# TinyMPC/TinyMPC

Measured on AMD Instinct MI355X. Metric: QP solves/sec (+ ADMM iters/sec), 64k-batch quadrotor hover, higher is better.
Workload: dtype f64; 1 GPU; quadrotor_hovering (nx=12, nu=4, N=10), 65536 identical instances per GPU, closed-loop MPC steps from a cold start (BASELINE configs[1]); batch_per_gpu=65536, total_batch=65536, parallelism=batch-sharded x1, mpc_steps_per_launch=8, stats_exchange=none (one rank), launcher=plain process

## Files before the change

tinympc_amd/csrc/admm_kernel.hip.h:

```cpp
#pragma once
#include <hip/hip_runtime.h>
#include <stdint.h>

namespace tinympc_amd {

enum : int {
    TAB_MB = 0,
    TAB_MF1 = 256,
    TAB_MF2 = 512,
    TAB_PT = 768,
    TAB_VEC = 1024,
    TAB_BOUNDS = 1024 + 16 * 16,
};
enum : int {
    VEC_CB = 0,
    VEC_CF = 1,
    VEC_QR = 2,
    VEC_SMASK = 3,
    VEC_NIM = 4,
    VEC_SOCFLAG = 5,
    VEC_CONE_BASE = 6,
    VEC_CONE_MU = 7,
    VEC_LINFLAG = 9,
    VEC_TLINFLAG = 10,
    VEC_COUNT = 16,
};
enum : int { LIN_KMAX = 4, LIN_KMAX_BIG = 32 };
enum : int {
    ATAB_AT = 0,
    ATAB_DK = 256,
    ATAB_DP = 512,
    ATAB_DC1 = 768,
    ATAB_DC2 = 1024,
    ATAB_DOUBLES = 1280,
};
// ... 293 lines not shown
    return r;
}
__device__ __forceinline__ double pinned_sub64(double a, double b) {
    double r = a - b;
    asm volatile("" : "+v"(r));
    return r;
}
__device__ __forceinline__ double vclamp64(double lo, double hi, double t) {
    double r;
    asm("v_max_f64 %0, %1, %2\n\tv_min_f64 %0, %3, %0" : "=&v"(r) : "v"(lo), "v"(t), "v"(hi));
    return r;
}

__device__ __forceinline__ double vmax_abs64(double a, double b) {
    double r;
    asm("v_max_f64 %0, %1, |%2|" : "=v"(r) : "v"(a), "v"(b));
    return r;
}
template <bool OPAQUE>
__device__ __forceinline__ double resid_max(double a, double b) {
    if constexpr (OPAQUE) return vmax_abs64(a, b);
    else return fmax(a, fabs(b));
}

#ifndef TINYMPC_PRIM_STORE
#define TINYMPC_PRIM_STORE 1
#endif
#ifndef TINYMPC_REF_LOAD
#define TINYMPC_REF_LOAD 1
#endif
#ifndef TINYMPC_FULL_LINE_STORES
#define TINYMPC_FULL_LINE_STORES 2
#endif
__device__ __forceinline__ double load_ref(const double* p) {
#if TINYMPC_REF_LOAD == 1
    return __builtin_nontemporal_load(p);
#else
    return *p;
#endif
}
__device__ __forceinline__ void store_primal(double* p, double v) {
#if TINYMPC_PRIM_STORE == 1
    __builtin_nontemporal_store(v, p);
#elif TINYMPC_PRIM_STORE == 2
    asm volatile("global_store_dwordx2 %0, %1, off sc1" : : "v"(p), "v"(v) : "memory");
#elif TINYMPC_PRIM_STORE == 3
    asm volatile("global_store_dwordx2 %0, %1, off sc0 sc1" : : "v"(p), "v"(v) : "memory");
#elif TINYMPC_PRIM_STORE == 4
    asm volatile("global_store_dwordx2 %0, %1, off sc0 sc1 nt" : : "v"(p), "v"(v) : "memory");
#else
    *p = v;
#endif
}

__device__ __forceinline__ double grp_max16(double v) {
#pragma unroll
    for (int off = 8; off >= 1; off >>= 1) v = fmax(v, __shfl_xor(v, off, 16));
    return v;
}
template <int W>
__device__ __forceinline__ double grp_maxw(double v) {
#pragma unroll
    for (int off = W / 2; off >= 1; off >>= 1) v = fmax(v, __shfl_xor(v, off, W));
    return v;
}

// ... 95 lines not shown
            double cv = 0.0;
#pragma unroll
            for (int r = 0; r < NF; ++r) { const double pr = tk[k * LW_ + R0 + r] * z[r]; cv = cv + pr; }
            const double bk = tk[KMAX_ * LW_ + k * LW_ + R0];
            if (cv > bk) {
                const double dist = (cv - bk) / tk[2 * KMAX_ * LW_ + k * LW_ + R0];
#pragma unroll
                for (int r = 0; r < NF; ++r) { const double pr = dist * tk[k * LW_ + R0 + r]; z[r] = z[r] - pr; }
            }
        }
#pragma unroll
        for (int r = 0; r < NF; ++r) { pv[at + r] = z[r]; pg[at + r] = t0[r] - z[r]; }
    }
}

template <int NX, int NU, int N, bool SOC, bool DBG, int MODE, int LIN = 0, bool HET = false, int KMAX = LIN_KMAX, bool ADAPT = false, bool UB = false, bool HALF = false,
          bool PF = false>
__global__ __launch_bounds__(64)
__attribute__((amdgpu_waves_per_eu(LIN != 0 ? solve_kernel_lin_waves(NX, NU, N, SOC, LIN, KMAX, UB) : solve_kernel_waves_per_simd(NX + NU, N, SOC, false, ADAPT),
                                   LIN != 0 ? solve_kernel_lin_waves(NX, NU, N, SOC, LIN, KMAX, UB) : solve_kernel_waves_per_simd(NX + NU, N, SOC, false, ADAPT))))
void admm_solve_kernel(const SolveArgs P) {
    constexpr bool LS = (LIN & 1) != 0, LT = (LIN & 2) != 0;
    constexpr int NZ = NX + NU;
    static_assert(NZ <= 16, "one instance per 16-lane DPP row");
    constexpr bool FUSED = MODE == 2 && LIN == 0 && fused_shape(NX, NU);
    static_assert(!HALF || (NZ <= 8 && FUSED && !SOC && !DBG && !HET && !ADAPT), "half rows: nx+nu <= 8, the plain box kernel on its fused step blocks");
    static_assert(!PF || (MODE == 2 && !SOC && !DBG && LIN == 0 && !HET && !ADAPT), "prefetch form: the plain box kernel");
    constexpr int RL = HALF ? 8 : 16;
    constexpr int IPW = 64 / RL;
    constexpr int RECD = N * NZ;
    constexpr int PF_PIECES = (IPW * RECD * 8 + 1023) / 1024;
    constexpr int PF_ARR = PF_PIECES * 128;
    constexpr unsigned long long RMASK = HALF ? 0xFFull : 0xFFFFull;
    const int lane = threadIdx.x & 63;
    const int j = lane & (RL - 1);
    const int grp = lane / RL;
    const bool is_state = j < NX;
    const bool is_input = (j >= NX) && (j < NZ);

    __shared__ double sPt[NX * 16];
    __shared__ double sLo[UB ? 1 : N * 16];
    __shared__ double sHi[UB ? 1 : N * 16];
    __shared__ double sLin[LS ? 3 * KMAX * 16 : 1];
    __shared__ double sTLin[LT ? 3 * N * KMAX * 16 : 1];
#ifndef TINYMPC_SOC_PD
#define TINYMPC_SOC_PD 2
#endif
    constexpr int SPD = TINYMPC_SOC_PD, SPR = SPD + 1;
    constexpr int CS = SOC ? ((NZ + 1) | 1) : 1;
    constexpr int SLOT_D = 3 * CS;
    constexpr int PL_GC = CS, PL_VC = 2 * CS;
    __shared__ double sC[SOC ? (4 * N + 1) * SLOT_D : 1];
    __shared__ double sP[ADAPT ? 4 * NX * NX : 1];
    constexpr int AKC = NX > NU ? NX : NU;
    constexpr bool HA = HET && ADAPT;
    __shared__ double sTab[(ADAPT && !HET) ? 3 * 16 * AKC : 1];
    __shared__ double sDl[ADAPT ? 4 * ADAPT_LOG : 1];
    if constexpr (ADAPT && !HET)
        for (int e = lane; e < 3 * 16 * AKC; e += 64) {
            const int t = e / (16 * AKC), r = e % (16 * AKC);
            sTab[e] = P.atab[t * 256 + (r % AKC) * 16 + r / AKC];
        }
    if constexpr (LS) for (int e = lane; e < 3 * KMAX * 16; e += 64) sLin[e] = P.tab[TAB_BOUNDS + 2 * N * 16 + e];
    if constexpr (LT) for (int e = lane; e < 3 * N * KMAX * 16; e += 64) sTLin[e] = P.tab[TAB_BOUNDS + 2 * N * 16 + 3 * KMAX * 16 + e];
    for (int e = lane; e < NX * 16; e += 64) sPt[e] = P.tab[TAB_PT + e];
    for (int e = lane; e < N * 16; e += 64) {
        if constexpr (!UB) {
            sLo[e] = P.tab[TAB_BOUNDS + e];
            sHi[e] = P.tab[TAB_BOUNDS + N * 16 + e];
        }
    }
    double mb[NZ], mf1[NX], mf2[NU];
#pragma unroll
    for (int k = 0; k < NZ; ++k) mb[k] = P.tab[TAB_MB + k * 16 + j];
#pragma unroll
// ... 32 lines not shown
            int t = p * 16 + j;
            item_at[p] = 4 * N * SLOT_D; item_mu[p] = 1.0f;
            if (heads && p * 16 < soc_items_of(heads, NX, N)) soc_passes = p + 1;
            for (unsigned m = heads; m; m &= m - 1) {
                const int hb = __builtin_ctz(m);
                const int cnt = hb < NX ? N : N - 1;
                if (t >= 0 && t < cnt) {
                    item_at[p] = (grp * N + t + (hb < NX ? 0 : 1)) * SLOT_D + hb;
                    item_mu[p] = (float)P.tab[TAB_VEC + VEC_CONE_MU * 16 + hb];
                    t = -1;
                } else if (t >= 0) t -= cnt;
            }
            item_rmu[p] = 1.0f / item_mu[p];
            const unsigned mb_ = __float_as_uint(item_mu[p]);
            const bool p2 = (mb_ & 0x807FFFFFu) == 0u && (mb_ >> 23) >= 127u - 60u && (mb_ >> 23) <= 127u + 60u;
            if (__builtin_amdgcn_ballot_w64(!p2) != 0ull) mu_pow2 = false;
        }
    }
    bool lin_lane = false, tlin_lane = false;
    if constexpr (LS) lin_lane = P.tab[TAB_VEC + VEC_LINFLAG * 16 + j] != 0.0;
    if constexpr (LT) tlin_lane = P.tab[TAB_VEC + VEC_TLINFLAG * 16 + j] != 0.0;
    constexpr bool LPL = solve_kernel_lin_planes(NX, NU, N, SOC, LIN, KMAX, UB);
    constexpr bool LSP = LS && LPL, LTP = LT && LPL, LSR = LS && !LPL, LTR = LT && !LPL;
    constexpr int CSL = LPL ? ((NZ + 1) | 1) : 1;
    __shared__ double sLV[LSP ? 4 * N * CSL : 1], sLG[LSP ? 4 * N * CSL : 1];
    __shared__ double sTV[LTP ? 4 * N * CSL : 1], sTG[LTP ? 4 * N * CSL : 1];
    double ones[(LSR || LTR) ? 16 : 1];
#pragma unroll
    for (int k = 0; k < ((LSR || LTR) ? 16 : 1); ++k) ones[k] = 1.0;
    bool lin_x_on = false, lin_u_on = false, tlin_x_on = false, tlin_u_on = false;
    if constexpr (LS) { lin_x_on = P.tab[TAB_VEC + VEC_LINFLAG * 16] != 0.0; lin_u_on = P.tab[TAB_VEC + VEC_LINFLAG * 16 + NX] != 0.0; }
    if constexpr (LT) { tlin_x_on = P.tab[TAB_VEC + VEC_TLINFLAG * 16] != 0.0; tlin_u_on = P.tab[TAB_VEC + VEC_TLINFLAG * 16 + NX] != 0.0; }
    double rho = P.rho;
    __builtin_amdgcn_fence(__ATOMIC_RELEASE, "wavefront");
    __builtin_amdgcn_wave_barrier();

    const double lo_u = P.tab[TAB_BOUNDS + (N > 1 ? 16 : 0) + j], hi_u = P.tab[TAB_BOUNDS + N * 16 + (N > 1 ? 16 : 0) + j];
    const double lo_u0 = P.tab[TAB_BOUNDS + j], hi_u0 = P.tab[TAB_BOUNDS + N * 16 + j];
    const int ninst = PF ? P.batch : (P.index ? *P.count : (P.perm ? P.perm_count : P.batch));
    const int ntiles = (ninst + IPW - 1) / IPW;
    const bool resumed = !PF && P.index != nullptr;
    const bool has_traj = !PF && P.traj != nullptr;
    extern __shared__ __attribute__((aligned(16))) double sPF[];
    typedef const __attribute__((address_space(1))) void* pf_gptr;
    typedef __attribute__((address_space(3))) void* pf_lptr;
    constexpr int PF_S0 = 128, PF_S1 = PF_S0 + PF_ARR, PF_S2 = PF_S1 + PF_ARR, PF_S3 = PF_S2 + PF_ARR;
    auto pf_issue = [&](const int t) {
        const int tl = P.reverse ? ntiles - 1 - t : t;
        __builtin_amdgcn_global_load_lds((pf_gptr)(P.x0 + ((size_t)tl * (IPW * NX) + (size_t)lane * 2)), (pf_lptr)sPF, 16, 0, 0);
        const size_t t0 = (size_t)tl * (IPW * RECD) + (size_t)lane * 2;
        auto arr = [&](const double* p, const int at) {
#pragma unroll
            for (int q = 0; q < PF_PIECES; ++q) __builtin_amdgcn_global_load_lds((pf_gptr)(p + t0 + q * 128), (pf_lptr)(sPF + at + q * 128), 16, 0, 0);
        };
        if (!P.cold) { arr(P.slack, PF_S0); arr(P.dual, PF_S1); arr(P.slack_prev, PF_S2); }
        if (P.pf_mask & 8) arr(P.ref, P.cold ? PF_S0 : PF_S3);
    };
    unsigned pf_ticket = 0u;
    const int pf_shard = PF ? (int)(blockIdx.x % (unsigned)(P.pf_shards > 0 ? P.pf_shards : 1)) : 0;
    typedef __attribute__((address_space(1))) unsigned* pf_ctr_t;
    unsigned long long pf_ctr_bits = PF ? (unsigned long long)(P.pf_counter + 16 * pf_shard) : 0ull;
    if constexpr (PF) asm volatile("" : "+v"(pf_ctr_bits));
    const pf_ctr_t pf_ctr = (pf_ctr_t)pf_ctr_bits;
    auto pf_draw = [&]() { return lane == 0 ? __hip_atomic_fetch_add(pf_ctr, 1u, __ATOMIC_RELAXED, __HIP_MEMORY_SCOPE_AGENT) : 0u; };
    const unsigned pf_base = PF ? P.pf_base[pf_shard] : 0u;
    int pf_next = 0, pf_i = 0;
// ... 87 lines not shown
            const double* het = nullptr;
            if constexpr (HET) {
                het = P.het_tabs + (size_t)b * TAB_BOUNDS;
#pragma unroll
                for (int k = 0; k < NZ; ++k) mb[k] = het[TAB_MB + k * 16 + j];
#pragma unroll
                for (int k = 0; k < NX; ++k) mf1[k] = het[TAB_MF1 + k * 16 + j];
#pragma unroll
                for (int k = 0; k < NU; ++k) mf2[k] = het[TAB_MF2 + (NX + k) * 16 + j];
                cb = het[TAB_VEC + VEC_CB * 16 + j];
                cf = het[TAB_VEC + VEC_CF * 16 + j];
                qr = het[TAB_VEC + VEC_QR * 16 + j];
                rho = het[TAB_VEC + 8 * 16 + j];
            }
            if constexpr (ADAPT) {
                rho = P.arho[b];
                const double* aK = P.aK + (size_t)b * (NU * NX);
                if (is_state) {
#pragma unroll
                    for (int k = 0; k < NU; ++k) mb[NX + k] = -aK[k + NU * j];
#pragma unroll
                    for (int k = 0; k < NX; ++k) sP[grp * NX * NX + k + NX * j] = P.aP[(size_t)b * (NX * NX) + k + NX * j];
                } else if (is_input) {
#pragma unroll
                    for (int k = 0; k < NX; ++k) mf1[k] = -aK[(j - NX) + NU * k];
                }
                __builtin_amdgcn_fence(__ATOMIC_RELEASE, "wavefront");
                __builtin_amdgcn_wave_barrier();
            }
            const double* atab_i = nullptr;
            if constexpr (HET && ADAPT) atab_i = P.atab + (size_t)b * ATAB_DOUBLES;
            (void)atab_i;
            const size_t lbase = (size_t)b * (N * NZ) + j - (is_input ? NZ : 0);
            double X[N], G[N], VN[N], VP[N], QX[N], Dn[N - 1];
            const int cw = grp * N * SLOT_D + (j < NZ ? j : NZ);
            const double x0v_in = is_state ? (PF ? pf_x0 : P.x0[(size_t)b * NX + j]) : 0.0;
            const int cl = grp * N * CSL + (j < NZ ? j : NZ);
            double VL[LSR ? N : 1], GL[LSR ? N : 1], VT[LTR ? N : 1], GT[LTR ? N : 1];
            double Qd[DBG ? N : 1], Pd[DBG ? N : 1], Dd[DBG ? N : 1];
            double ref_last = 0.0, qx_last_plain = 0.0;
#pragma unroll
            for (int s = 0; s < N; ++s) {
                const bool valid = is_state || (is_input && s >= 1);
                const size_t off = lbase + s * NZ;
                const bool warm = valid && !P.cold;
                if constexpr (PF) {
                    VN[s] = warm ? pfVN[s] : 0.0;
                    G[s] = warm ? pfG[s] : 0.0;
                    VP[s] = warm ? pfVP[s] : 0.0;
                    QX[s] = pfQXs[s];
                    X[s] = 0.0;
                    if (s == N - 1) ref_last = pf_rl;
                    continue;
                }
                const double r = valid ? (P.ref_shared ? P.ref[off - (size_t)b * (N * NZ)] : load_ref(P.ref + off)) : 0.0;
                VN[s] = warm ? P.slack[off] : 0.0;
                G[s] = warm ? P.dual[off] : 0.0;
                VP[s] = warm ? P.slack_prev[off] : 0.0;
                QX[s] = -(r * qr);
                X[s] = 0.0;
                if (s == N - 1) ref_last = r;
                if constexpr (SOC) {
                    double vc0 = (warm && soc_lane) ? (resumed ? P.cslack : P.prim)[off] : 0.0;
                    const double gc0 = (warm && soc_lane) ? P.cdual[off] : 0.0;
                    if (s == 0 && is_state && soc_lane && !resumed) vc0 = x0v_in;
                    sC[cw + s * SLOT_D] = vc0 - gc0;
                    sC[cw + s * SLOT_D + PL_GC] = gc0;
                    sC[cw + s * SLOT_D + PL_VC] = vc0;
                }
                if constexpr (LS) {
                    const double vl0 = (warm && lin_lane) ? (resumed ? P.lslack : P.prim)[off] : 0.0;
                    const double gl0 = (warm && lin_lane) ? P.ldual[off] : 0.0;
                    if constexpr (LSP) { sLV[cl + s * CSL] = vl0; sLG[cl + s * CSL] = gl0; } else { VL[s] = vl0; GL[s] = gl0; }
                }
                if constexpr (LT) {
                    const double vt0 = (warm && tlin_lane) ? (resumed ? P.tlslack : P.prim)[off] : 0.0;
                    const double gt0 = (warm && tlin_lane) ? P.tldual[off] : 0.0;
                    if constexpr (LTP) { sTV[cl + s * CSL] = vt0; sTG[cl + s * CSL] = gt0; } else { VT[s] = vt0; GT[s] = gt0; }
                }
                if constexpr (DBG) { Qd[s] = 0.0; Pd[s] = 0.0; Dd[s] = 0.0; }
            }
            double x0v = x0v_in;
            auto terminal_term = [&]() {
                double pt[NX];
#pragma unroll
                for (int k = 0; k < NX; ++k)
                    pt[k] = ADAPT ? sP[grp * NX * NX + k + NX * (is_state ? j : 0)] : (HET ? het[TAB_PT + k * 16 + j] : sPt[k * 16 + j]);
                double xp = 0.0;
                if constexpr (HALF) ring1_half<0, NX>(xp, ref_last, pt);
                else xp = ring_sum<MODE, 0, NX>(0.0, ref_last, pt);
                qx_last_plain = QX[N - 1];
// ... 3 lines not shown
            auto flush_c = [&](int n) {
                __builtin_amdgcn_fence(__ATOMIC_RELEASE, "wavefront");
                __builtin_amdgcn_wave_barrier();
                if (P.aC2 && is_state) {
                    double* c2 = P.aC2 + (size_t)b * (NX * NX) + NX * j;
                    double v[NX], d[NX];
#pragma unroll
                    for (int k = 0; k < NX; ++k) { v[k] = c2[k]; d[k] = P.atab[(HA ? (size_t)b * ATAB_DOUBLES : (size_t)0) + ATAB_DC2 + k * 16 + j]; }
                    for (int i = 0; i < n; ++i) {
                        const double dl = sDl[grp * ADAPT_LOG + i];
#pragma unroll
                        for (int k = 0; k < NX; ++k) v[k] = taylor_step(v[k], dl, d[k]);
                    }
#pragma unroll
                    for (int k = 0; k < NX; ++k) c2[k] = v[k];
                }
                if (P.aC1 && j < NU) {
                    double* c1 = P.aC1 + (size_t)b * (NU * NU) + NU * j;
                    double v[NU], d[NU];
#pragma unroll
                    for (int k = 0; k < NU; ++k) { v[k] = c1[k]; d[k] = P.atab[(HA ? (size_t)b * ATAB_DOUBLES : (size_t)0) + ATAB_DC1 + k * 16 + j]; }
                    for (int i = 0; i < n; ++i) {
                        const double dl = sDl[grp * ADAPT_LOG + i];
#pragma unroll
                        for (int k = 0; k < NU; ++k) v[k] = taylor_step(v[k], dl, d[k]);
                    }
#pragma unroll
                    for (int k = 0; k < NU; ++k) c1[k] = v[k];
                }
            };
            if (!has_traj && !(PF && P.ref_shared)) terminal_term();
            const int traj_k0 = has_traj ? (P.traj_step0 + (P.traj_offsets ? P.traj_offsets[b] : 0)) : 0;

            int iter = 0, solved = 0, checked = 0;
            unsigned acc_iter = 0, acc_solved = 0;
            bool vp_touched = false;
            double rp = 0.0, rd = 0.0;
            const int nsteps = PF ? 1 : (P.steps > 1 ? P.steps : 1);
            const int iter_first = resumed ? P.iter_base : 0;
            for (int step = 0; step < nsteps; ++step) {
                X[0] = x0v;
                if (has_traj) {
                    if (is_state) {
#pragma unroll
                        for (int s = 0; s < N; ++s) {
                            int kk = traj_k0 + step + s;
                            kk = kk < P.traj_points ? kk : P.traj_points - 1;
                            const double r = P.traj[(size_t)kk * NX + j];
                            QX[s] = -(r * qr);
                            if (s == N - 1) ref_last = r;
                        }
                    }
                    terminal_term();
                }
                if (P.reset_duals) {
#pragma unroll
                    for (int s = 0; s < N; ++s) G[s] = 0.0;
                }
                if constexpr (SOC) {
                    if (step > 0) {
#pragma unroll
                        for (int s = 0; s < N; ++s) {
                            const double vc0 = soc_lane ? X[s] : 0.0;
                            sC[cw + s * SLOT_D] = vc0 - sC[cw + s * SLOT_D + PL_GC];
                            sC[cw + s * SLOT_D + PL_VC] = vc0;
                        }
                    }
                }
                if constexpr (LS) {
                    if (step > 0) {
#pragma unroll
                        for (int s = 0; s < N; ++s) { if constexpr (LSP) sLV[cl + s * CSL] = lin_lane ? X[s] : 0.0; else VL[s] = lin_lane ? X[s] : 0.0; }
                    } else if (is_state && lin_lane && !resumed) { if constexpr (LSP) sLV[cl] = x0v; else VL[0] = x0v; }
                }
                if constexpr (LT) {
                    if (step > 0) {
#pragma unroll
                        for (int s = 0; s < N; ++s) { if constexpr (LTP) sTV[cl + s * CSL] = tlin_lane ? X[s] : 0.0; else VT[s] = tlin_lane ? X[s] : 0.0; }
                    } else if (is_state && tlin_lane && !resumed) { if constexpr (LTP) sTV[cl] = x0v; else VT[0] = x0v; }
                }
                if constexpr (LPL) __builtin_amdgcn_fence(__ATOMIC_RELEASE, "wavefront");
                const int iter0 = iter_first;
                iter = iter0; solved = 0;
                if (resumed && P.check_termination > 0) checked = 1;
                int countdown = P.check_termination;
                double wr[SOC ? SPR : 1];
                bool gcz[SOC_PASSES];
#pragma unroll
                for (int p = 0; p < SOC_PASSES; ++p) gcz[p] = false;
                if constexpr (SOC) {
#pragma unroll
                    for (int d = 1; d <= SPR && d <= N; ++d) wr[(N - d) % SPR] = sC[cw + (N - d) * SLOT_D];
                }
                for (int it = iter0; it < P.max_iter; ++it) {
                    double lvr[LSP ? SPR : 1], lgr[LSP ? SPR : 1], tvr[LTP ? SPR : 1], tgr[LTP ? SPR : 1];
                    if constexpr (LPL) {
#pragma unroll
                        for (int d = 1; d <= SPR && d <= N; ++d) {
                            if constexpr (LSP) { lvr[(N - d) % SPR] = sLV[cl + (N - d) * CSL]; lgr[(N - d) % SPR] = sLG[cl + (N - d) * CSL]; }
                            if constexpr (LTP) { tvr[(N - d) % SPR] = sTV[cl + (N - d) * CSL]; tgr[(N - d) % SPR] = sTG[cl + (N - d) * CSL]; }
                        }
                    }
                    auto lin_w = [&](const int s_) { if constexpr (LSP) return lvr[s_ % SPR] - lgr[s_ % SPR]; else return VL[LSR ? s_ : 0] - GL[LSR ? s_ : 0]; };
                    auto tlin_w = [&](const int s_) { if constexpr (LTP) return tvr[s_ % SPR] - tgr[s_ % SPR]; else return VT[LTR ? s_ : 0] - GT[LTR ? s_ : 0]; };
                    double qhi;
                    {
                        double t = fma(-rho, VN[N - 1] - G[N - 1], QX[N - 1]);
                        if constexpr (SOC) t = fma(-rho, wr[(N - 1) % SPR], t);
                        if constexpr (LS) t = fma(-rho, lin_w(N - 1), t);
                        if constexpr (LT) t = fma(-rho, tlin_w(N - 1), t);
                        qhi = t;
                        if constexpr (DBG) {
                            double ql = fma(-rho, VN[N - 1] - G[N - 1], qx_last_plain);
                            if constexpr (SOC) ql = fma(-rho, wr[(N - 1) % SPR], ql);
                            if constexpr (LS) ql = fma(-rho, lin_w(N - 1), ql);
                            if constexpr (LT) ql = fma(-rho, tlin_w(N - 1), ql);
                            Qd[N - 1] = is_state ? ql : t;
                            Pd[N - 1] = t;
// ... 13 lines not shown
                            pcur = res;
                            qhi = qlo;
                        }
                        Dn[0] = fma(pcur, nim, cf);
                    }
#pragma unroll
                    for (int i = N - 2; i >= 0 && !HALF; --i) {
                        if constexpr (SOC) {
                            if (i >= SPD) wr[(i - SPD) % SPR] = sC[cw + (i - SPD) * SLOT_D];
                        }
                        if constexpr (LSP) { if (i >= SPD) { lvr[(i - SPD) % SPR] = sLV[cl + (i - SPD) * CSL]; lgr[(i - SPD) % SPR] = sLG[cl + (i - SPD) * CSL]; } }
                        if constexpr (LTP) { if (i >= SPD) { tvr[(i - SPD) % SPR] = sTV[cl + (i - SPD) * CSL]; tgr[(i - SPD) % SPR] = sTG[cl + (i - SPD) * CSL]; } }
                        if constexpr (SOC || LPL) __builtin_amdgcn_sched_barrier(0);
                        if constexpr (FUSED) {
                            double qlo, res;
                            if constexpr (SOC) fused_backward_step_soc<NX, NU>(qlo, res, VN[i], G[i], QX[i], wr[i % SPR], rho, smask, cb, pcur, qhi, mb, mb + NX);
                            else fused_backward_step<NX, NU>(qlo, res, VN[i], G[i], QX[i], rho, smask, cb, pcur, qhi, mb, mb + NX);
                            pcur = res;
                            Dn[i] = fma(res, nim, cf);
                            if constexpr (DBG) { Qd[i] = qlo; Pd[i] = res; Dd[i + 1] = res; }
                            qhi = qlo;
                            continue;
                        }
                        double qlo = fma(-rho, VN[i] - G[i], QX[i]);
                        if constexpr (SOC) qlo = fma(-rho, wr[i % SPR], qlo);
                        if constexpr (LS) qlo = fma(-rho, lin_w(i), qlo);
                        if constexpr (LT) qlo = fma(-rho, tlin_w(i), qlo);
                        const double res = ring_sum2<MODE, NX, NU>(fma(qlo, smask, cb), pcur, mb, qhi, mb + NX);
                        pcur = res;
                        Dn[i] = fma(res, nim, cf);
                        if constexpr (DBG) { Qd[i] = qlo; Pd[i] = res; Dd[i + 1] = res; }
                        qhi = qlo;
                    }
                    constexpr bool LAZY_RES = N <= 12;
                    constexpr bool TIGHT = FUSED && !HALF && LAZY_RES && !SOC && NX % 4 == 0;
                    double pmax = 0.0, dmax = 0.0;
                    auto slot_update = [&](const int s, const double lo, const double hi, const double gcv, const double glv, const double gtv) {
                        const double xi = X[s];
                        const double t = xi + G[s];
                        const double vn = TIGHT ? vclamp64(lo, hi, t) : vmin64(hi, vmax64(lo, t));
                        if constexpr (!LAZY_RES) {
                            pmax = resid_max<true>(pmax, xi - vn);
                            dmax = resid_max<true>(dmax, VP[s] - vn);
                        }
                        G[s] = t - vn;
                        VN[s] = vn;
                        if constexpr (SOC) {
                            sC[cw + s * SLOT_D] = fma(xi, socmask, gcv);
                        }
                        if constexpr (LSP) sLV[cl + s * CSL] = (lin_lane && (is_state || s >= 1)) ? (xi + glv) : 0.0;
                        if constexpr (LTP) sTV[cl + s * CSL] = (tlin_lane && (is_state || s >= 1)) ? (xi + gtv) : 0.0;
                        if constexpr (LSR || LTR) {
                            auto halfspaces = [&](double z, const double* tabk, const int nk) {
                                for (int k = 0; k < nk; ++k) {
                                    const double a = tabk[k * 16 + j];
                                    const double bk = tabk[KMAX * 16 + k * 16 + j];
                                    const double nn = tabk[2 * KMAX * 16 + k * 16 + j];
                                    const double prod = a * z;
                                    double cs = 0.0, ci = 0.0;
                                    ring1<0, NX>(cs, prod, ones);
                                    ring1<NX, NU>(ci, prod, ones);
                                    const double cv = is_state ? cs : ci;
                                    if (cv > bk) z = z - ((cv - bk) / nn) * a;
                                }
                                return z;
                            };
                            if constexpr (LSR) {
                                const bool on = lin_lane && (is_state || s >= 1);
// ... 62 lines not shown
                                tt_d = tt; vn_d = vn;
                            } else G[i] = tt - vn;
                            VN[i] = vn;
                            if constexpr (SOC) sC[cw + i * SLOT_D] = fma(xi, socmask, gr[i % SPR]);
                            lo_c = lo_n; hi_c = hi_n;
                            continue;
                        }
                        const double t = ring_sum<MODE, 0, NX>(Dn[i], X[i], mf1);
                        X[i + 1] = ring_short<MODE, NX, NU>(t, t, mf2);
                        slot_update(i, lo_c, hi_c, gr[SOC ? i % SPR : 0], glr[LSP ? i % SPR : 0], gtr[LTP ? i % SPR : 0]);
                        lo_c = lo_n; hi_c = hi_n;
                    }
                    if constexpr (TIGHT && N >= 2) G[N - 2] = tt_d - vn_d;
                    (void)tt_d; (void)vn_d;
                    slot_update(N - 1, lo_c, hi_c, gr[SOC ? (N - 1) % SPR : 0], glr[LSP ? (N - 1) % SPR : 0], gtr[LTP ? (N - 1) % SPR : 0]);
                    if constexpr (LPL) {
                        __builtin_amdgcn_fence(__ATOMIC_RELEASE, "wavefront");
                        __builtin_amdgcn_wave_barrier();
                        if constexpr (LSP) {
                            if (lin_x_on) project_halfspace_columns<NX, KMAX, 16, 16>(j, grp, N, CSL, 0, 0, sLV, sLG, sLin, 0, P.n_lin);
                            if (lin_u_on) project_halfspace_columns<NU, KMAX, 16, 16>(j, grp, N, CSL, NX, 1, sLV, sLG, sLin, 0, P.n_lin);
                        }
                        if constexpr (LTP) {
                            if (tlin_x_on) project_halfspace_columns<NX, KMAX, 16, 16>(j, grp, N, CSL, 0, 0, sTV, sTG, sTLin, 3 * KMAX * 16, P.n_tlin);
                            if (tlin_u_on) project_halfspace_columns<NU, KMAX, 16, 16>(j, grp, N, CSL, NX, 1, sTV, sTG, sTLin, 3 * KMAX * 16, P.n_tlin);
                        }
                        __builtin_amdgcn_fence(__ATOMIC_RELEASE, "wavefront");
                        __builtin_amdgcn_wave_barrier();
                    }
                    bool conv = false;
                    auto termination = [&]() {
                        if (countdown > 0 && --countdown == 0) {
                            countdown = P.check_termination;
                            checked = 1;
                            constexpr int PS0 = N >= 2 ? 1 : 0, PS1 = N - 1;
                            auto lost = [&](const int s) {
                                return (int)(fabs(X[s] - VN[s]) >= P.tol_pri) | (int)(fabs(VP[s] - VN[s]) * rho >= P.tol_dua);
                            };
                            const bool maybe = ((int)!(rho > 0.0) | (int)!(lost(PS0) | lost(PS1))) != 0;
                            unsigned long long fold = __ballot(maybe);
                            fold &= fold >> 1; fold &= fold >> 2; fold &= fold >> 4;
                            if constexpr (!HALF) fold &= fold >> 8;
                            const bool any_row = (fold & (HALF ? 0x0101010101010101ull : 0x0001000100010001ull)) != 0ull;
                            const bool last_test = (P.max_iter - 1 - it) < P.check_termination;
                            if (last_test || any_row) {
                                if constexpr (LAZY_RES) {
#pragma unroll
                                    for (int s = 0; s < N; ++s) {
                                        pmax = resid_max<false>(pmax, X[s] - VN[s]);
                                        dmax = resid_max<false>(dmax, VP[s] - VN[s]);
                                    }
                                }
                                rp = pmax;
                                rd = dmax * rho;
                                const bool ok = (rp < P.tol_pri) && (rd < P.tol_dua);
                                const unsigned long long bal = __ballot(ok);
                                conv = ((bal >> (grp * RL)) & RMASK) == RMASK;
                            }
                        }
                    };
                    if constexpr (SOC) {
                        __builtin_amdgcn_fence(__ATOMIC_RELEASE, "wavefront");
                        __builtin_amdgcn_wave_barrier();
                        double n0 = sC[item_at[0]], n1 = sC[item_at[0] + 1], n2 = sC[item_at[0] + 2];
#pragma unroll
                        for (int d = 1; d <= SPR && d <= N; ++d) wr[(N - d) % SPR] = sC[cw + (N - d) * SLOT_D];
                        termination();
                        bool any_exact = false;
#pragma unroll
                        for (int p = 0; p < SOC_PASSES; ++p) {
                            if (p > 0 && p >= soc_passes) break;
                            const int at = item_at[p];
                            if (p > 0) { n0 = sC[at]; n1 = sC[at + 1]; n2 = sC[at + 2]; }
                            const double s0 = n0, s1 = n1, s2 = n2;
                            if (soc_all_inside(s0, s1, s2, item_mu[p])) {
                                sC[at + PL_VC] = s0; sC[at + PL_VC + 1] = s1; sC[at + PL_VC + 2] = s2;
                                if (!gcz[p]) {
                                    sC[at + PL_GC] = 0.0; sC[at + PL_GC + 1] = 0.0; sC[at + PL_GC + 2] = 0.0;
                                    gcz[p] = true;
                                }
                            } else {
                                double r0, r1, r2;
                                soc_project3(s0, s1, s2, item_mu[p], item_rmu[p], mu_pow2, r0, r1, r2);
                                const double g0 = s0 - r0, g1 = s1 - r1, g2 = s2 - r2;
                                sC[at + PL_VC] = r0; sC[at + PL_VC + 1] = r1; sC[at + PL_VC + 2] = r2;
                                sC[at + PL_GC] = g0; sC[at + PL_GC + 1] = g1; sC[at + PL_GC + 2] = g2;
                                sC[at] = r0 - g0; sC[at + 1] = r1 - g1; sC[at + 2] = r2 - g2;
                                gcz[p] = false;
                                any_exact = true;
                            }
                        }
                        if (it == iter0 && !proj_lane) {
#pragma unroll
                            for (int s = 0; s < N; ++s) sC[cw + s * SLOT_D + PL_GC] = 0.0;
                        }
                        __builtin_amdgcn_fence(__ATOMIC_RELEASE, "wavefront");
                        __builtin_amdgcn_wave_barrier();
                        if (any_exact) {
#pragma unroll
                            for (int d = 1; d <= SPR && d <= N; ++d) wr[(N - d) % SPR] = sC[cw + (N - d) * SLOT_D];
                        }
                    }
                    iter += 1;
                    if constexpr (ADAPT) {
                        if (it > 0 && it % 5 == 0) {
                            double at[NX];
#pragma unroll
                            for (int k = 0; k < NX; ++k) at[k] = HA ? atab_i[ATAB_AT + k * 16 + j] : sTab[j * AKC + k];
                            double pri_res = 0.0, ax_max = 0.0, z_max = 0.0, dual_res = 0.0, px_max = 0.0, aty_max = 0.0, q_max = 0.0;
                            double pxq_max = 0.0;
#pragma unroll
                            for (int i = 0; i < N - 1; ++i) {
                                const double axs = ring_sum<MODE, 0, NX>(0.0, X[i], mf1);
                                const double dyn = ring_short<MODE, NX, NU>(axs, is_input ? X[i + 1] : 0.0, mf2) - X[i + 1];
                                const double a = is_state ? dyn : X[i + 1];
                                const double zz = VN[i + 1];
                                const bool on = is_state || is_input;
                                pri_res = fmax(pri_res, on ? fabs(a - zz) : 0.0);
                                ax_max = fmax(ax_max, on ? fabs(a) : 0.0);
                                z_max = fmax(z_max, on ? fabs(zz) : 0.0);
                                const double init = is_state ? (i >= 1 ? -G[i] : 0.0) : G[i + 1];
                                const double aty = ring_sum<MODE, 0, NX>(init, G[i + 1], at);
                                const double xs = is_state ? X[i] : X[i + 1];
                                const double px = qr * xs;
                                dual_res = fmax(dual_res, on ? fabs((px + px) + aty) : 0.0);
                                pxq_max = fmax(pxq_max, on ? fabs(px) : 0.0);
                                aty_max = fmax(aty_max, on ? fabs(aty) : 0.0);
                            }
                            {
                                double prow[NX];
#pragma unroll
                                for (int k = 0; k < NX; ++k) prow[k] = sP[grp * NX * NX + (is_state ? j : 0) + NX * k];
                                const double pxl = ring_sum<MODE, 0, NX>(0.0, X[N - 1], prow);
                                const double ql = qr * X[N - 1];
                                const double atyl = -G[N - 1];
                                dual_res = fmax(dual_res, is_state ? fabs((pxl + ql) + atyl) : 0.0);
// ... 6 lines not shown
                            const double pri_norm = fmax(ax_max, z_max);
                            const double dual_norm = fmax(fmax(px_max, aty_max), q_max);
                            const double eps = 1e-10;
                            const double normalized_pri = pri_res / (pri_norm + eps);
                            const double normalized_dual = dual_res / (dual_norm + eps);
                            const double ratio = normalized_pri / (normalized_dual + eps);
                            double new_rho = rho * sqrt(ratio);
                            if (P.aclip) new_rho = fmin(fmax(new_rho, P.arho_min), P.arho_max);
                            const double delta = new_rho - rho;
                            if (is_state) {
#pragma unroll
                                for (int k = 0; k < NU; ++k) mb[NX + k] = -taylor_step(-mb[NX + k], delta, (HA ? atab_i[ATAB_DK + k * 16 + j] : sTab[(16 + j) * AKC + k]));
#pragma unroll
                                for (int k = 0; k < NX; ++k) {
                                    const int e = grp * NX * NX + k + NX * j;
                                    sP[e] = taylor_step(sP[e], delta, (HA ? atab_i[ATAB_DP + k * 16 + j] : sTab[(32 + j) * AKC + k]));
                                }
                            } else if (is_input) {
#pragma unroll
                                for (int k = 0; k < NX; ++k) mf1[k] = -taylor_step(-mf1[k], delta, (HA ? atab_i[ATAB_DK + k * 16 + j] : sTab[(16 + j) * AKC + k]));
                            }
                            if (P.aC1 || P.aC2) {
                                if (j == 0) sDl[grp * ADAPT_LOG + ndl] = delta;
                                if (++ndl == ADAPT_LOG) { flush_c(ndl); ndl = 0; }
                            }
                            rho = new_rho;
                            __builtin_amdgcn_fence(__ATOMIC_RELEASE, "wavefront");
                            __builtin_amdgcn_wave_barrier();
                            QX[N - 1] = qx_last_plain;
                            terminal_term();
                        }
                    }
                    if constexpr (!SOC) termination();
                    if (conv) { solved = 1; break; }
#pragma unroll
                    for (int s = 0; s < N; ++s) VP[s] = VN[s];
                    vp_touched = true;
                }
                acc_iter += (unsigned)(iter - iter0);
                acc_solved += (unsigned)solved;
                if (P.iter_log && j == 0) P.iter_log[(size_t)step * P.batch + b] = solved ? iter : -iter;
                if (P.u0_log && is_input) P.u0_log[((size_t)step * P.batch + b) * NU + (j - NX)] = X[1];
                if (nsteps > 1) {
                    x0v = is_state ? X[1] : 0.0;
                }
            }

            constexpr bool FLS = TINYMPC_FULL_LINE_STORES != 0 && (PF || TINYMPC_FULL_LINE_STORES == 2) && !SOC && LIN == 0 && !DBG;
            if (FLS && (P.store_mask & 32) == 0) {
                if constexpr (FLS) {
                    const size_t seg = (size_t)b * (N * NZ) + j;
                    const bool in_row = j < NZ;
#pragma unroll
                    for (int s = 0; s < N; ++s) {
                        const size_t off = seg + s * NZ;
                        const double xs = is_input ? (s + 1 < N ? X[s + 1 < N ? s + 1 : s] : 0.0) : X[s];
                        const double vs = is_input ? (s + 1 < N ? VN[s + 1 < N ? s + 1 : s] : 0.0) : VN[s];
                        const double gs = is_input ? (s + 1 < N ? G[s + 1 < N ? s + 1 : s] : 0.0) : G[s];
                        const double ps = is_input ? (s + 1 < N ? VP[s + 1 < N ? s + 1 : s] : 0.0) : VP[s];
                        if (in_row) {
                            if (P.store_mask & 1) {
                                if (acc_iter > 0) { if constexpr (PF) P.prim[off] = xs; else store_primal(P.prim + off, xs); }
                                else if (s == 0 && is_state) P.prim[off] = xs;
                            }
                            if (P.store_mask & 2) P.slack[off] = vs;
                            if (P.store_mask & 4) P.dual[off] = gs;
                            if ((P.store_mask & 8) && vp_touched) P.slack_prev[off] = ps;
                        }
                    }
                }
            } else
#pragma unroll
            for (int s = 0; s < N; ++s) {
                const bool valid = is_state || (is_input && s >= 1);
                const size_t off = lbase + s * NZ;
                if (valid) {
                    if (((P.store_mask & 1) || ((P.store_mask & 32) && s <= 1)) && (acc_iter > 0 || (s == 0 && is_state))) {
                        if constexpr (SOC || LIN != 0) P.prim[off] = X[s];
                        else store_primal(P.prim + off, X[s]);
                    }
                    if (P.store_mask & 2) P.slack[off] = VN[s];
                    if (P.store_mask & 4) P.dual[off] = G[s];
                    if ((P.store_mask & 8) && vp_touched) P.slack_prev[off] = VP[s];
                    if constexpr (SOC) {
                        if (soc_lane && (P.store_mask & 16)) {
                            P.cslack[off] = sC[cw + s * SLOT_D + ((proj_lane || iter <= iter_first) ? PL_VC : 0)];
                            P.cdual[off] = sC[cw + s * SLOT_D + PL_GC];
                        }
                    }
                    if constexpr (LSP) { if (lin_lane && (P.store_mask & 16)) { P.lslack[off] = sLV[cl + s * CSL]; P.ldual[off] = sLG[cl + s * CSL]; } }
                    if constexpr (LTP) { if (tlin_lane && (P.store_mask & 16)) { P.tlslack[off] = sTV[cl + s * CSL]; P.tldual[off] = sTG[cl + s * CSL]; } }
                    if constexpr (LSR) { if (lin_lane && (P.store_mask & 16)) { P.lslack[off] = VL[s]; P.ldual[off] = GL[s]; } }
                    if constexpr (LTR) { if (tlin_lane && (P.store_mask & 16)) { P.tlslack[off] = VT[s]; P.tldual[off] = GT[s]; } }
                    if constexpr (DBG) {
                        if (P.dbg_qr && acc_iter > 0) {
                            P.dbg_qr[off] = Qd[s];
                            P.dbg_pd[off] = is_state ? Pd[s] : Dd[s];
                        }
                    }
                }
            }
            if constexpr (ADAPT) {
                if (ndl > 0) flush_c(ndl);
                if (j == 0) P.arho[b] = rho;
                if (is_state) {
#pragma unroll
                    for (int k = 0; k < NU; ++k) P.aK[(size_t)b * (NU * NX) + k + NU * j] = -mb[NX + k];
#pragma unroll
                    for (int k = 0; k < NX; ++k) P.aP[(size_t)b * (NX * NX) + k + NX * j] = sP[grp * NX * NX + k + NX * j];
                }
            }
            if (P.x0_next && acc_iter > 0 && is_state) P.x0_next[(size_t)b * NX + j] = X[1];
            const double ps = grp_maxw<RL>(is_state ? rp : 0.0), pi = grp_maxw<RL>(is_input ? rp : 0.0);
            const double ds = grp_maxw<RL>(is_state ? rd : 0.0), di = grp_maxw<RL>(is_input ? rd : 0.0);
            if (P.next_index) {
                const bool open = j == 0 && !solved;
                const unsigned long long m = __ballot(open);
                if (m) {
                    const int first = __ffsll((long long)m) - 1;
                    int at = 0;
                    if (lane == first) at = atomicAdd(P.next_count, __popcll(m));
                    at = __shfl(at, first);
                    if (open) P.next_index[at + __popcll(m & ((1ull << lane) - 1ull))] = b;
                }
            }
            if (j == 0) {
                P.status[b] = make_int4(iter, solved, solved ? 1 : 11, checked);
                double4 rr = make_double4(ps, pi, ds, di);
                *reinterpret_cast<double4*>(P.resid + (size_t)b * 4) = rr;
                if (P.accum) {
                    if constexpr (PF) {
                        __hip_atomic_fetch_add(&P.accum[b].x, acc_iter, __ATOMIC_RELAXED, __HIP_MEMORY_SCOPE_AGENT);
                        __hip_atomic_fetch_add(&P.accum[b].y, acc_solved, __ATOMIC_RELAXED, __HIP_MEMORY_SCOPE_AGENT);
                    } else {
                        uint2 ac = P.accum[b];
                        ac.x += acc_iter;
                        ac.y += acc_solved;
                        P.accum[b] = ac;
                    }
                }
            }
        }
    }
}

}
```

Measured before the change: 2.866 billion QP solves/s.

## Shadow previous-slack in LDS and streamline termination bookkeeping in short-horizon kernel

Moves the previous-iteration slack array VP out of registers into a per-lane LDS shadow, keeping only the two probe stages in registers. This cuts VGPR pressure, which could allow more waves per SIMD. The termination probe now builds per-condition ballot masks and compares against a precomputed dual threshold (tol_dua/rho, rounded up two ulps) instead of multiplying by rho. Iteration and solved counts are derived once after the loop rather than updated every iteration. In exchange each iteration adds LDS stores, and full residual checks now need LDS loads.

```diff
diff --git a/tinympc_amd/csrc/admm_kernel.hip.h b/tinympc_amd/csrc/admm_kernel.hip.h
--- a/tinympc_amd/csrc/admm_kernel.hip.h
+++ b/tinympc_amd/csrc/admm_kernel.hip.h
@@ -1,6 +1,30 @@
 #pragma once
+#ifndef TINYMPC_HOST_ONLY
 #include <hip/hip_runtime.h>
 #include <stdint.h>
+#define TINYMPC_HD __host__ __device__
+#else
+#define TINYMPC_HD
+#endif
+
+namespace tinympc_amd {
+
+TINYMPC_HD inline double probe_step_up(double x) {
+    if (!(x < __builtin_inf())) return x;
+    long long b;
+    __builtin_memcpy(&b, &x, 8);
+    b = x == 0.0 ? 1ll : (x > 0.0 ? b + 1 : b - 1);
+    __builtin_memcpy(&x, &b, 8);
+    return x;
+}
+TINYMPC_HD inline double dual_probe_threshold(double tol_dua, double rho) {
+    if (!(rho > 0.0)) return __builtin_nan("");
+    const double thr = probe_step_up(probe_step_up(tol_dua / rho));
+    return thr < __builtin_inf() ? thr : __builtin_nan("");
+}
+
+}
+#ifndef TINYMPC_HOST_ONLY
 
 namespace tinympc_amd {
 
@@ -360,6 +384,21 @@
 #ifndef TINYMPC_FULL_LINE_STORES
 #define TINYMPC_FULL_LINE_STORES 2
 #endif
+#ifndef TINYMPC_VPREV_SHADOW
+#define TINYMPC_VPREV_SHADOW 1
+#endif
+#ifndef TINYMPC_SCALAR_BOOKKEEPING
+#define TINYMPC_SCALAR_BOOKKEEPING 1
+#endif
+#ifndef TINYMPC_SHADOW_BATCHES
+#define TINYMPC_SHADOW_BATCHES 1
+#endif
+#ifndef TINYMPC_PROBE_MASKS
+#define TINYMPC_PROBE_MASKS 1
+#endif
+#ifndef TINYMPC_PROBE_THRESHOLD
+#define TINYMPC_PROBE_THRESHOLD 1
+#endif
 __device__ __forceinline__ double load_ref(const double* p) {
 #if TINYMPC_REF_LOAD == 1
     return __builtin_nontemporal_load(p);
@@ -521,6 +560,14 @@
     constexpr int PF_PIECES = (IPW * RECD * 8 + 1023) / 1024;
     constexpr int PF_ARR = PF_PIECES * 128;
     constexpr unsigned long long RMASK = HALF ? 0xFFull : 0xFFFFull;
+    constexpr bool LAZY_RES = N <= 12;
+    constexpr bool TIGHT = FUSED && !HALF && LAZY_RES && !SOC && NX % 4 == 0;
+    constexpr bool SHORT = TIGHT && !PF;
+    constexpr bool SHADOW = SHORT && TINYMPC_VPREV_SHADOW != 0;
+    constexpr bool PROBE_MASKS = SHORT && TINYMPC_PROBE_MASKS != 0;
+    constexpr bool SBK = SHORT && TINYMPC_SCALAR_BOOKKEEPING != 0;
+    constexpr bool PROBE_THR = SHORT && !ADAPT && !HET && TINYMPC_PROBE_THRESHOLD != 0;
+    constexpr int PS0 = N >= 2 ? 1 : 0, PS1 = N - 1;
     const int lane = threadIdx.x & 63;
     const int j = lane & (RL - 1);
     const int grp = lane / RL;
@@ -530,6 +577,7 @@
     __shared__ double sPt[NX * 16];
     __shared__ double sLo[UB ? 1 : N * 16];
     __shared__ double sHi[UB ? 1 : N * 16];
+    __shared__ double sVP[SHADOW ? N * 64 : 1];
     __shared__ double sLin[LS ? 3 * KMAX * 16 : 1];
     __shared__ double sTLin[LT ? 3 * N * KMAX * 16 : 1];
 #ifndef TINYMPC_SOC_PD
@@ -628,6 +676,12 @@
     if constexpr (LS) { lin_x_on = P.tab[TAB_VEC + VEC_LINFLAG * 16] != 0.0; lin_u_on = P.tab[TAB_VEC + VEC_LINFLAG * 16 + NX] != 0.0; }
     if constexpr (LT) { tlin_x_on = P.tab[TAB_VEC + VEC_TLINFLAG * 16] != 0.0; tlin_u_on = P.tab[TAB_VEC + VEC_TLINFLAG * 16 + NX] != 0.0; }
     double rho = P.rho;
+    double thr_dua = 0.0;
+    if constexpr (PROBE_THR) {
+        const double t = dual_probe_threshold(P.tol_dua, P.rho);
+        thr_dua = __hiloint2double(__builtin_amdgcn_readfirstlane(__double2hiint(t)), __builtin_amdgcn_readfirstlane(__double2loint(t)));
+    }
+    (void)thr_dua;
     __builtin_amdgcn_fence(__ATOMIC_RELEASE, "wavefront");
     __builtin_amdgcn_wave_barrier();
 
@@ -781,7 +835,15 @@
             if constexpr (HET && ADAPT) atab_i = P.atab + (size_t)b * ATAB_DOUBLES;
             (void)atab_i;
             const size_t lbase = (size_t)b * (N * NZ) + j - (is_input ? NZ : 0);
-            double X[N], G[N], VN[N], VP[N], QX[N], Dn[N - 1];
+            double X[N], G[N], VN[N], VP[SHADOW ? 1 : N], QX[N], Dn[N - 1];
+            double VPp[2] = {0.0, 0.0};
+            int lane_a = lane, lane_b = lane, lane_c = lane;
+            if constexpr (SHADOW) { asm volatile("" : "+v"(lane_a)); asm volatile("" : "+v"(lane_b)); asm volatile("" : "+v"(lane_c)); }
+            double* const svp_in = sVP + lane_a;
+            double* const svp = sVP + lane_b;
+            double* const svp_out = sVP + lane_c;
+            auto vprev = [&](const int s) { if constexpr (SHADOW) return svp_out[s * 64]; else return VP[s]; };
+            (void)VPp; (void)svp; (void)svp_in; (void)svp_out;
             const int cw = grp * N * SLOT_D + (j < NZ ? j : NZ);
             const double x0v_in = is_state ? (PF ? pf_x0 : P.x0[(size_t)b * NX + j]) : 0.0;
             const int cl = grp * N * CSL + (j < NZ ? j : NZ);
@@ -805,7 +867,12 @@
                 const double r = valid ? (P.ref_shared ? P.ref[off - (size_t)b * (N * NZ)] : load_ref(P.ref + off)) : 0.0;
                 VN[s] = warm ? P.slack[off] : 0.0;
                 G[s] = warm ? P.dual[off] : 0.0;
-                VP[s] = warm ? P.slack_prev[off] : 0.0;
+                const double vp_in = warm ? P.slack_prev[off] : 0.0;
+                if constexpr (SHADOW) {
+                    svp_in[s * 64] = vp_in;
+                    if (s == PS0) VPp[0] = vp_in;
+                    if (s == PS1) VPp[1] = vp_in;
+                } else VP[s] = vp_in;
                 QX[s] = -(r * qr);
                 X[s] = 0.0;
                 if (s == N - 1) ref_last = r;
@@ -875,6 +942,9 @@
             if (!has_traj && !(PF && P.ref_shared)) terminal_term();
             const int traj_k0 = has_traj ? (P.traj_step0 + (P.traj_offsets ? P.traj_offsets[b] : 0)) : 0;
 
+            unsigned long long rho_bad = 0ull;
+            if constexpr (PROBE_MASKS) rho_bad = __builtin_amdgcn_ballot_w64(!(rho > 0.0));
+            (void)rho_bad;
             int iter = 0, solved = 0, checked = 0;
             unsigned acc_iter = 0, acc_solved = 0;
             bool vp_touched = false;
@@ -927,6 +997,8 @@
                 iter = iter0; solved = 0;
                 if (resumed && P.check_termination > 0) checked = 1;
                 int countdown = P.check_termination;
+                int iter_conv = iter0;
+                (void)iter_conv;
                 double wr[SOC ? SPR : 1];
                 bool gcz[SOC_PASSES];
 #pragma unroll
@@ -1006,8 +1078,6 @@
                         if constexpr (DBG) { Qd[i] = qlo; Pd[i] = res; Dd[i + 1] = res; }
                         qhi = qlo;
                     }
-                    constexpr bool LAZY_RES = N <= 12;
-                    constexpr bool TIGHT = FUSED && !HALF && LAZY_RES && !SOC && NX % 4 == 0;
                     double pmax = 0.0, dmax = 0.0;
                     auto slot_update = [&](const int s, const double lo, const double hi, const double gcv, const double glv, const double gtv) {
                         const double xi = X[s];
@@ -1136,19 +1206,47 @@
                     auto termination = [&]() {
                         if (countdown > 0 && --countdown == 0) {
                             countdown = P.check_termination;
-                            checked = 1;
-                            constexpr int PS0 = N >= 2 ? 1 : 0, PS1 = N - 1;
+                            if constexpr (!SBK) checked = 1;
+                            auto vpr = [&](const int s) { if constexpr (SHADOW) return VPp[s == PS0 ? 0 : 1]; else return VP[s]; };
                             auto lost = [&](const int s) {
-                                return (int)(fabs(X[s] - VN[s]) >= P.tol_pri) | (int)(fabs(VP[s] - VN[s]) * rho >= P.tol_dua);
+                                if constexpr (PROBE_THR) return (int)(fabs(X[s] - VN[s]) >= P.tol_pri) | (int)(fabs(vpr(s) - VN[s]) >= thr_dua);
+                                else return (int)(fabs(X[s] - VN[s]) >= P.tol_pri) | (int)(fabs(vpr(s) - VN[s]) * rho >= P.tol_dua);
                             };
-                            const bool maybe = ((int)!(rho > 0.0) | (int)!(lost(PS0) | lost(PS1))) != 0;
-                            unsigned long long fold = __ballot(maybe);
+                            unsigned long long fold;
+                            if constexpr (PROBE_MASKS) {
+                                auto lost_m = [&](const int s) {
+                                    const unsigned long long lp = __builtin_amdgcn_ballot_w64(fabs(X[s] - VN[s]) >= P.tol_pri);
+                                    if constexpr (PROBE_THR) return lp | __builtin_amdgcn_ballot_w64(fabs(vpr(s) - VN[s]) >= thr_dua);
+                                    else return lp | __builtin_amdgcn_ballot_w64(fabs(vpr(s) - VN[s]) * rho >= P.tol_dua);
+                                };
+                                if constexpr (ADAPT) rho_bad = __builtin_amdgcn_ballot_w64(!(rho > 0.0));
+                                fold = (rho_bad | ~(lost_m(PS0) | lost_m(PS1))) & __builtin_amdgcn_ballot_w64(true);
+                            } else {
+                                const bool maybe = ((int)!(rho > 0.0) | (int)!(lost(PS0) | lost(PS1))) != 0;
+                                fold = __ballot(maybe);
+                            }
                             fold &= fold >> 1; fold &= fold >> 2; fold &= fold >> 4;
                             if constexpr (!HALF) fold &= fold >> 8;
                             const bool any_row = (fold & (HALF ? 0x0101010101010101ull : 0x0001000100010001ull)) != 0ull;
                             const bool last_test = (P.max_iter - 1 - it) < P.check_termination;
                             if (last_test || any_row) {
-                                if constexpr (LAZY_RES) {
+                                if constexpr (SHADOW) {
+                                    auto half = [&](const int s0, const int s1) {
+                                        double vp[N];
+#pragma unroll
+                                        for (int s = s0; s < s1; ++s) vp[s] = s == PS0 ? VPp[0] : (s == PS1 ? VPp[1] : svp[s * 64]);
+                                        __builtin_amdgcn_sched_barrier(0);
+                                        __builtin_amdgcn_s_waitcnt(0xc07f);
+                                        __builtin_amdgcn_sched_barrier(0);
+#pragma unroll
+                                        for (int s = s0; s < s1; ++s) {
+                                            pmax = resid_max<false>(pmax, X[s] - VN[s]);
+                                            dmax = resid_max<false>(dmax, vp[s] - VN[s]);
+                                        }
+                                    };
+                                    if constexpr (TINYMPC_SHADOW_BATCHES == 1) half(0, N);
+                                    else { half(0, (N + 1) / 2); half((N + 1) / 2, N); }
+                                } else if constexpr (LAZY_RES) {
 #pragma unroll
                                     for (int s = 0; s < N; ++s) {
                                         pmax = resid_max<false>(pmax, X[s] - VN[s]);
@@ -1157,9 +1255,23 @@
                                 }
                                 rp = pmax;
                                 rd = dmax * rho;
-                                const bool ok = (rp < P.tol_pri) && (rd < P.tol_dua);
-                                const unsigned long long bal = __ballot(ok);
-                                conv = ((bal >> (grp * RL)) & RMASK) == RMASK;
+                                unsigned one = 1u;
+                                if constexpr (SBK) asm volatile("" : "+v"(one));
+                                (void)one;
+                                unsigned long long bal;
+                                if constexpr (PROBE_MASKS) bal = __builtin_amdgcn_ballot_w64(rp < P.tol_pri) & __builtin_amdgcn_ballot_w64(rd < P.tol_dua);
+                                else {
+                                    const bool ok = (rp < P.tol_pri) && (rd < P.tol_dua);
+                                    bal = __ballot(ok);
+                                }
+                                if constexpr (SBK) {
+                                    int seen = it + 1;
+                                    asm volatile("" : "+v"(seen));
+                                    iter_conv = seen;
+                                    const int all_ok = (int)((((unsigned)(bal >> (grp * RL)) & (unsigned)RMASK) + one) >> RL);
+                                    solved = all_ok;
+                                    conv = all_ok != 0;
+                                } else conv = ((bal >> (grp * RL)) & RMASK) == RMASK;
                             }
                         }
                     };
@@ -1205,7 +1317,7 @@
                             for (int d = 1; d <= SPR && d <= N; ++d) wr[(N - d) % SPR] = sC[cw + (N - d) * SLOT_D];
                         }
                     }
-                    iter += 1;
+                    if constexpr (!SBK) iter += 1;
                     if constexpr (ADAPT) {
                         if (it > 0 && it % 5 == 0) {
                             double at[NX];
@@ -1278,10 +1390,21 @@
                         }
                     }
                     if constexpr (!SOC) termination();
-                    if (conv) { solved = 1; break; }
-#pragma unroll
-                    for (int s = 0; s < N; ++s) VP[s] = VN[s];
+                    if constexpr (SBK) { if (conv) break; }
+                    else if (conv) { solved = 1; break; }
+                    if constexpr (SHADOW) {
+#pragma unroll
+                        for (int s = 0; s < N; ++s) svp[s * 64] = VN[s];
+                        VPp[0] = VN[PS0]; VPp[1] = VN[PS1];
+                    } else {
+#pragma unroll
+                        for (int s = 0; s < N; ++s) VP[s] = VN[s];
+                    }
                     vp_touched = true;
+                }
+                if constexpr (SBK) {
+                    iter = solved ? iter_conv : (P.max_iter > iter0 ? P.max_iter : iter0);
+                    if (P.check_termination > 0 && (solved || P.max_iter - iter0 >= P.check_termination)) checked = 1;
                 }
                 acc_iter += (unsigned)(iter - iter0);
                 acc_solved += (unsigned)solved;
@@ -1303,7 +1426,7 @@
                         const double xs = is_input ? (s + 1 < N ? X[s + 1 < N ? s + 1 : s] : 0.0) : X[s];
                         const double vs = is_input ? (s + 1 < N ? VN[s + 1 < N ? s + 1 : s] : 0.0) : VN[s];
                         const double gs = is_input ? (s + 1 < N ? G[s + 1 < N ? s + 1 : s] : 0.0) : G[s];
-                        const double ps = is_input ? (s + 1 < N ? VP[s + 1 < N ? s + 1 : s] : 0.0) : VP[s];
+                        const double ps = is_input ? (s + 1 < N ? vprev(s + 1 < N ? s + 1 : s) : 0.0) : vprev(s);
                         if (in_row) {
                             if (P.store_mask & 1) {
                                 if (acc_iter > 0) { if constexpr (PF) P.prim[off] = xs; else store_primal(P.prim + off, xs); }
@@ -1327,7 +1450,7 @@
                     }
                     if (P.store_mask & 2) P.slack[off] = VN[s];
                     if (P.store_mask & 4) P.dual[off] = G[s];
-                    if ((P.store_mask & 8) && vp_touched) P.slack_prev[off] = VP[s];
+                    if ((P.store_mask & 8) && vp_touched) P.slack_prev[off] = vprev(s);
                     if constexpr (SOC) {
                         if (soc_lane && (P.store_mask & 16)) {
                             P.cslack[off] = sC[cw + s * SLOT_D + ((proj_lane || iter <= iter_first) ? PL_VC : 0)];
@@ -1391,3 +1514,4 @@
 }
 
 }
+#endif
```

Result: slower. 2.473 billion QP solves/s (-13.7%).
